# mit-han-lab/distrifuser

Measured on AMD Instinct MI355X. Metric: end-to-end latency (s) per image, SDXL 50-step DDIM, lower is better.
Workload: dtype bf16; 1 GPU; model=sdxl-base (random init), global_batch=1, image=3840x3840, seq_len=230400, scheduler=ddim, steps_per_image=50, parallelism=patch1, mode=corrected_async_gn, cuda_graph=True

## Files before the change

distrifuser_amd/csrc/bindings.hip:

```cpp

#include <torch/extension.h>
#include <ATen/hip/HIPContext.h>
#include <c10/hip/HIPStream.h>

#include <array>

#include "kernels.h"

namespace {

int dtype_of(const at::Tensor& t) {
    switch (t.scalar_type()) {
        case at::kBFloat16: return DFA_BF16;
        case at::kHalf: return DFA_F16;
        case at::kFloat: return DFA_F32;
        default: TORCH_CHECK(false, "unsupported dtype ", t.scalar_type());
    }
}

bool is_b16(const at::Tensor& t) {
    return t.scalar_type() == at::kBFloat16 || t.scalar_type() == at::kHalf;
}

hipStream_t cur_stream() { return at::hip::getCurrentHIPStream().stream(); }

at::Tensor b16_param(const at::Tensor& t, const at::Tensor& ref, const char* op,
                     const char* name) {
    TORCH_CHECK(t.scalar_type() == ref.scalar_type() || !is_b16(t), op, ": ", name,
                " must have x's dtype (", ref.scalar_type(), "), got ", t.scalar_type());
    return t.to(ref.scalar_type()).contiguous();
}

at::Tensor gn_partial_stats(const at::Tensor& x, int64_t group_len, int ngt) {
    auto partial = at::zeros({2, (long)ngt}, x.options().dtype(at::kFloat));
    launch_gn_stats_partial(x.data_ptr(), partial.data_ptr<float>(), group_len, ngt,
                            dtype_of(x), cur_stream());
    return partial;
}

const void* gn_affine(const c10::optional<at::Tensor>& t, const at::Tensor& x, at::Tensor& keep) {
    if (!t.has_value()) return nullptr;
    keep = t->to(x.scalar_type()).contiguous();
    return keep.data_ptr();
}

at::Tensor group_norm_stats(const at::Tensor& x_, int64_t num_groups) {
    TORCH_CHECK(x_.is_cuda() && x_.dim() == 4, "x must be CUDA [N,C,H,W]");
    auto x = x_.contiguous();
    const int64_t n = x.size(0), c = x.size(1), hw = x.size(2) * x.size(3);
    TORCH_CHECK(c % num_groups == 0);
    const int64_t group_len = (c / num_groups) * hw;
    const int ngt = (int)(n * num_groups);
    auto partial = gn_partial_stats(x, group_len, ngt);
    auto out = at::empty({2, n, num_groups, 1, 1, 1}, x.options());
    launch_gn_finalize(partial.data_ptr<float>(), out.data_ptr(), 1.0f / (float)group_len, ngt,
                       dtype_of(x), cur_stream());
    return out;
}

at::Tensor group_norm_apply(const at::Tensor& x_, const at::Tensor& mean_,
                            const at::Tensor& meansq_, const c10::optional<at::Tensor>& w_,
                            const c10::optional<at::Tensor>& b_, double eps, bool silu) {
    TORCH_CHECK(x_.is_cuda() && x_.dim() == 4);
    auto x = x_.contiguous();
    const int64_t n = x.size(0), c = x.size(1), hw = x.size(2) * x.size(3);
    auto mean = mean_.to(at::kFloat).contiguous().view({-1});
    auto meansq = meansq_.to(at::kFloat).contiguous().view({-1});
    TORCH_CHECK(mean.numel() % n == 0);
    const int g = (int)(mean.numel() / n);
    TORCH_CHECK(c % g == 0, "channels ", c, " not divisible by groups ", g);
    at::Tensor w, b;
    const void* wp = gn_affine(w_, x, w);
    const void* bp = gn_affine(b_, x, b);
    auto y = at::empty_like(x);
    launch_gn_apply(x.data_ptr(), y.data_ptr(), mean.data_ptr<float>(), meansq.data_ptr<float>(),
                    wp, bp, (float)eps, hw, (int)c, g, (int)n, silu, dtype_of(x), cur_stream());
    return y;
}

at::Tensor group_norm_silu(const at::Tensor& x_, int64_t num_groups,
                           const c10::optional<at::Tensor>& w_,
                           const c10::optional<at::Tensor>& b_, double eps, bool silu) {
    TORCH_CHECK(x_.is_cuda() && x_.dim() == 4);
    auto x = x_.contiguous();
    const int64_t n = x.size(0), c = x.size(1), hw = x.size(2) * x.size(3);
    TORCH_CHECK(c % num_groups == 0);
    const int64_t group_len = (c / num_groups) * hw;
    const int ngt = (int)(n * num_groups);
    auto partial = gn_partial_stats(x, group_len, ngt);
    auto moments = at::empty({2, (long)ngt}, x.options().dtype(at::kFloat));
    launch_gn_finalize(partial.data_ptr<float>(), moments.data_ptr(), 1.0f / (float)group_len,
                       ngt, DFA_F32, cur_stream());
    at::Tensor w, b;
    const void* wp = gn_affine(w_, x, w);
    const void* bp = gn_affine(b_, x, b);
    auto y = at::empty_like(x);
    launch_gn_apply(x.data_ptr(), y.data_ptr(), moments.data_ptr<float>(),
                    moments.data_ptr<float>() + ngt, wp, bp, (float)eps, hw, (int)c,
                    (int)num_groups, (int)n, silu, dtype_of(x), cur_stream());
    return y;
}

at::Tensor gn_merge_stats(const at::Tensor& buffer, int64_t slot_off, int64_t own,
                          const at::Tensor& fresh_, bool corrected) {
    TORCH_CHECK(buffer.is_cuda() && buffer.dim() == 2 && buffer.stride(1) == 1);
    auto fresh = fresh_.contiguous();
    const int ng = (int)(fresh.numel() / 2);
    TORCH_CHECK(fresh.scalar_type() == buffer.scalar_type());
    auto out = at::empty({2, (long)ng}, buffer.options().dtype(at::kFloat));
    launch_gn_merge_stats(buffer.data_ptr(), buffer.stride(0), slot_off,
                          (int)buffer.size(0), (int)own, fresh.data_ptr(),
                          out.data_ptr<float>(), ng, corrected, dtype_of(buffer),
                          cur_stream());
    return out;
}

at::Tensor geglu(const at::Tensor& h_) {
    TORCH_CHECK(h_.is_cuda());
    auto h = h_.contiguous();
    const int64_t inner = h.size(-1) / 2;
    TORCH_CHECK(h.size(-1) % 2 == 0);
    auto sizes = h.sizes().vec();
    sizes.back() = inner;
    auto out = at::empty(sizes, h.options());
    launch_geglu(h.data_ptr(), out.data_ptr(), h.numel() / (2 * inner), inner, dtype_of(h),
                 cur_stream());
    return out;
}

at::Tensor cfg_affine_step(const at::Tensor& noise, const at::Tensor& x, double g, double ca,
                           double cb) {
    TORCH_CHECK(noise.is_cuda() && noise.size(0) == 2);
    auto n = noise.contiguous();
// ... 334 lines not shown
    p.k = reinterpret_cast<const uint16_t*>(kc.data_ptr());
    p.v = reinterpret_cast<const uint16_t*>(vc.data_ptr());
    p.B = (int)qc.size(0);
    p.L = qc.size(1);
    p.sb = qc.stride(0);
    p.scale = 1.0f / std::sqrt(512.0f);
    auto o = at::empty_like(qc);
    p.o = reinterpret_cast<uint16_t*>(o.data_ptr());
    launch_vae_attention(p, dtype_of(q), cur_stream());
    return o;
}

std::vector<at::Tensor> mfma_probe(const at::Tensor& a, const at::Tensor& b) {
    TORCH_CHECK(a.is_cuda() && a.sizes() == (at::IntArrayRef{64, 8}));
    auto af = a.to(at::kFloat).contiguous(), bf = b.to(at::kFloat).contiguous();
    auto d = at::zeros({64, 4}, af.options());
    launch_mfma_probe(af.data_ptr<float>(), bf.data_ptr<float>(), d.data_ptr<float>(),
                      cur_stream());
    return {d};
}

std::vector<at::Tensor> mfma_probe32(const at::Tensor& a, const at::Tensor& b) {
    TORCH_CHECK(a.is_cuda() && a.sizes() == (at::IntArrayRef{64, 8}));
    auto af = a.to(at::kFloat).contiguous(), bf = b.to(at::kFloat).contiguous();
    auto d = at::zeros({64, 16}, af.options());
    launch_mfma_probe32(af.data_ptr<float>(), bf.data_ptr<float>(), d.data_ptr<float>(),
                        cur_stream());
    return {d};
}
}

PYBIND11_MODULE(TORCH_EXTENSION_NAME, m) {
    m.def("group_norm_stats", &group_norm_stats, "per-group moments [2,N,G,1,1,1]");
    m.def("group_norm_apply", &group_norm_apply, "normalize+affine(+SiLU) from given moments");
    m.def("group_norm_silu", &group_norm_silu, "fused GroupNorm(+SiLU)");
    m.def("geglu", &geglu, "a * gelu(gate) over last-dim halves");
    m.def("gn_merge_stats", &gn_merge_stats,
          "merge stale peer GN moments with fresh local ones (one launch)");
    m.def("cfg_affine_step", &cfg_affine_step, "fused CFG combine + affine scheduler update");
    m.def("flash_attention", &flash_attention, "bf16/fp16 flash attention (chunked stale KV)");
    m.def("flash_attention_ext", &flash_attention_ext,
          "flash attention with split-KV and optional log-sum-exp -> [out] or [out, lse]",
          pybind11::arg("q"), pybind11::arg("k"), pybind11::arg("v"),
          pybind11::arg("kv_splits") = 1, pybind11::arg("return_lse") = false);
    m.def("flash_attention_partial", &flash_attention_partial,
          "split-KV partials into caller buffers (o_part fp32 [S,B,Lq,H,D], lse_part [S,B,H,Lq])");
    m.def("merge_attention", &merge_attention,
          "merge fp32 attention partials by their log-sum-exp -> [out, lse]",
          pybind11::arg("o_parts"), pybind11::arg("lse_parts"), pybind11::arg("out_bf16") = true,
          pybind11::arg("out_dtype") = pybind11::none());
    m.def("cfg_dpm_step", &cfg_dpm_step, "fused CFG + DPM-Solver++(2M) update -> (prev, x0)");
    m.def("layer_norm", &layer_norm, "bf16/fp16 fused LayerNorm");
    m.def("add_layer_norm", &add_layer_norm, "bf16/fp16 fused residual-add + LayerNorm -> (sum, y)");
    m.def("vae_attention", &vae_attention, "bf16/fp16 single-head d=512 VAE mid attention");
    m.def("conv3x3", &conv3x3,
          "bf16/fp16 implicit-GEMM 3x3 conv, stride 1/2, in-place halo rows; pad_lo=0 "
          "(stride 2) pads bottom/right only",
          pybind11::arg("x"), pybind11::arg("wp"), pybind11::arg("bias"), pybind11::arg("cout"), pybind11::arg("stride"),
          pybind11::arg("top"), pybind11::arg("bot"), pybind11::arg("residual"), pybind11::arg("bias2"),
          pybind11::arg("pad_lo") = 1);
    m.def("mfma_probe", &mfma_probe, "dump mfma_f32_16x16x32_bf16 fragment mapping");
    m.def("mfma_probe32", &mfma_probe32, "dump mfma_f32_32x32x16_bf16 fragment mapping");
}
```

distrifuser_amd/csrc/groupnorm.hip:

```cpp

#include "common.h"
#include "kernels.h"
#include <algorithm>

namespace {

template <typename T, bool VEC>
__global__ void gn_stats_partial_kernel(const T* __restrict__ x, float* __restrict__ partial,
                                        int64_t group_len, int chunks, int ngt) {
    constexpr int V = VEC ? VecN<T>::value : 1;
    const int ng = blockIdx.x / chunks;
    const int chunk = blockIdx.x % chunks;
    const int64_t nvec = group_len / V;
    const int64_t per = (nvec + chunks - 1) / chunks;
    const int64_t v0 = chunk * per;
    const int64_t v1 = min(v0 + per, nvec);
    const T* base = x + (int64_t)ng * group_len;

    float s = 0.f, ss = 0.f;
    for (int64_t iv = v0 + threadIdx.x; iv < v1; iv += blockDim.x) {
        if (VEC) {
            uint4 raw = *reinterpret_cast<const uint4*>(base + iv * V);
            const T* e = reinterpret_cast<const T*>(&raw);
#pragma unroll
            for (int j = 0; j < V; ++j) {
                float f = to_f32(e[j]);
                s += f;
                ss += f * f;
            }
        } else {
            float f = to_f32(base[iv]);
            s += f;
            ss += f * f;
// ... 73 lines not shown
        gn_stats_partial_kernel<T, true><<<grid, 256, 0, stream>>>(
            reinterpret_cast<const T*>(x), partial, group_len, chunks, ngt);
    else
        gn_stats_partial_kernel<T, false><<<grid, 256, 0, stream>>>(
            reinterpret_cast<const T*>(x), partial, group_len, chunks, ngt);
}

template <typename T>
void gn_apply_t(const void* x, void* y, const float* mean, const float* meansq, const void* w,
                const void* b, float eps, int64_t hw, int C, int G, int N, bool silu,
                hipStream_t stream) {
    const int64_t total = (int64_t)N * C * hw;
    const bool vec = (hw % VecN<T>::value) == 0;
    const int block = 256;
    if (vec) {
        int grid = grid_for(total / VecN<T>::value, block);
        if (silu)
            gn_apply_kernel<T, true, true><<<grid, block, 0, stream>>>(
                (const T*)x, (T*)y, mean, meansq, (const T*)w, (const T*)b, eps, hw, C, G, total);
        else
            gn_apply_kernel<T, false, true><<<grid, block, 0, stream>>>(
                (const T*)x, (T*)y, mean, meansq, (const T*)w, (const T*)b, eps, hw, C, G, total);
    } else {
        int grid = grid_for(total, block);
        if (silu)
            gn_apply_kernel<T, true, false><<<grid, block, 0, stream>>>(
                (const T*)x, (T*)y, mean, meansq, (const T*)w, (const T*)b, eps, hw, C, G, total);
        else
            gn_apply_kernel<T, false, false><<<grid, block, 0, stream>>>(
                (const T*)x, (T*)y, mean, meansq, (const T*)w, (const T*)b, eps, hw, C, G, total);
    }
}

template <typename T, bool CORRECTED>
__global__ void gn_merge_stats_kernel(T* __restrict__ buffer, int64_t row_stride,
                                      int64_t slot_off, int n_peers, int own,
                                      const T* __restrict__ fresh, float* __restrict__ out,
                                      int ng) {
    const int g = blockIdx.x * blockDim.x + threadIdx.x;
    if (g >= ng) return;
    float m_sum = 0.f, q_sum = 0.f;
    float m_own = 0.f, q_own = 0.f;
    for (int p = 0; p < n_peers; ++p) {
        const T* slot = buffer + p * row_stride + slot_off;
        float m = to_f32(slot[g]);
        float q = to_f32(slot[ng + g]);
        if (p == own) {
            m_own = m;
            q_own = q;
            if (!CORRECTED) {
                m = to_f32(fresh[g]);
                q = to_f32(fresh[ng + g]);
            }
        }
        m_sum += m;
        q_sum += q;
    }
    float mean = m_sum / n_peers;
    float msq = q_sum / n_peers;
    const float f_m = to_f32(fresh[g]);
    const float f_q = to_f32(fresh[ng + g]);
    if (CORRECTED) {
        mean += f_m - m_own;
        msq += f_q - q_own;
        const float var = msq - mean * mean;
        if (var < 0.f) msq = mean * mean + (f_q - f_m * f_m);
// ... 58 lines not shown
void launch_gn_finalize(const float* partial, void* out, float inv_count, int ngt, int dtype,
                        hipStream_t stream) {
    int total = 2 * ngt;
    int block = 256;
    int grid = (total + block - 1) / block;
    switch (dtype) {
        case DFA_BF16:
            gn_finalize_kernel<bf16_t><<<grid, block, 0, stream>>>(partial, (bf16_t*)out, inv_count, ngt);
            break;
        case DFA_F16:
            gn_finalize_kernel<f16_t><<<grid, block, 0, stream>>>(partial, (f16_t*)out, inv_count, ngt);
            break;
        default:
            gn_finalize_kernel<float><<<grid, block, 0, stream>>>(partial, (float*)out, inv_count, ngt);
            break;
    }
}

void launch_gn_apply(const void* x, void* y, const float* mean, const float* meansq,
                     const void* weight, const void* bias, float eps, int64_t hw, int C, int G,
                     int N, bool silu, int dtype, hipStream_t stream) {
    switch (dtype) {
        case DFA_BF16:
            gn_apply_t<bf16_t>(x, y, mean, meansq, weight, bias, eps, hw, C, G, N, silu, stream);
            break;
        case DFA_F16:
            gn_apply_t<f16_t>(x, y, mean, meansq, weight, bias, eps, hw, C, G, N, silu, stream);
            break;
        default:
            gn_apply_t<float>(x, y, mean, meansq, weight, bias, eps, hw, C, G, N, silu, stream);
            break;
    }
}
```

distrifuser_amd/csrc/kernels.h:

```cpp
#pragma once

#include <hip/hip_runtime.h>
#include <cstdint>

enum DfaDtype : int { DFA_BF16 = 0, DFA_F16 = 1, DFA_F32 = 2 };

void launch_gn_stats_partial(const void* x, float* partial, int64_t group_len,
                             int n_groups_total, int dtype, hipStream_t stream);
void launch_gn_finalize(const float* partial, void* out, float inv_count,
                        int n_groups_total, int dtype, hipStream_t stream);
void launch_gn_apply(const void* x, void* y, const float* mean, const float* meansq,
                     const void* weight, const void* bias, float eps, int64_t hw,
                     int C, int G, int N, bool silu, int dtype, hipStream_t stream);

void launch_gn_merge_stats(void* buffer, int64_t row_stride, int64_t slot_off,
                           int n_peers, int own, const void* fresh, float* out,
                           int ng, bool corrected, int dtype, hipStream_t stream);

void launch_geglu(const void* in, void* out, int64_t rows, int64_t inner, int dtype,
                  hipStream_t stream);

void launch_cfg_affine_step(const void* noise_u, const void* noise_c, const void* x, void* out,
                            float g, float ca, float cb, int64_t total, int dtype,
                            hipStream_t stream);

struct Conv3x3Params {
    const uint16_t* x;
    const uint16_t* top;
    const uint16_t* bot;
    const uint16_t* wp;
    const uint16_t* bias;
    const uint16_t* residual;
    const uint16_t* bias2;
    uint16_t* o;
    int B, Cin, Cout, H, W, Ho, Wo;
    int KS, CT;
    int debug;
    int pad_lo;
    int64_t x_sb, x_sc;
    int64_t t_sb, t_sc;
    int64_t b_sb, b_sc;
};
void launch_conv3x3(const Conv3x3Params& p, int stride, int dtype, hipStream_t stream);

void launch_cfg_dpm_step(const void* nu, const void* nc, const void* x, const void* x0_prev,
                         void* out, void* x0_out, float g, float ca, float cb, float cc,
// ... 53 lines not shown
```

distrifuser_amd/models/transformer.py:

```python

from __future__ import annotations

import torch
from torch import nn

from .. import ops

from .layers import LayerFactory


class BasicTransformerBlock(nn.Module):
    def __init__(
        self,
        dim: int,
        heads: int,
        dim_head: int,
        cross_dim: int,
        *,
        factory: LayerFactory,
    ):
        super().__init__()
        self.norm1 = nn.LayerNorm(dim)
        self.attn1 = factory.self_attention(dim, heads, dim_head)
        self.norm2 = nn.LayerNorm(dim)
        self.attn2 = factory.cross_attention(dim, cross_dim, heads, dim_head)
        self.norm3 = nn.LayerNorm(dim)
        self.ff = factory.feed_forward(dim)

    def forward(self, x: torch.Tensor, encoder_hidden_states: torch.Tensor,
                pending=None):
        if pending is None:
            n1 = ops.layer_norm(x, self.norm1.weight, self.norm1.bias, self.norm1.eps)
        else:
            x, n1 = ops.add_layer_norm(x, pending, self.norm1.weight, self.norm1.bias,
                                       self.norm1.eps)
        x, h = ops.add_layer_norm(x, self.attn1(n1), self.norm2.weight, self.norm2.bias,
                                  self.norm2.eps)
        x, n3 = ops.add_layer_norm(x, self.attn2(h, encoder_hidden_states),
                                   self.norm3.weight, self.norm3.bias, self.norm3.eps)
        return x, self.ff(n3)


class Transformer2DModel(nn.Module):

    def __init__(
        self,
        channels: int,
        heads: int,
        dim_head: int,
        layers: int,
        cross_dim: int,
        *,
        factory: LayerFactory,
        groups: int = 32,
        use_linear_projection: bool = True,
    ):
        super().__init__()
        inner = heads * dim_head
        self.use_linear_projection = use_linear_projection
        self.norm = factory.group_norm(groups, channels, eps=1e-6, fuse_silu=False)
        if use_linear_projection:
            self.proj_in = nn.Linear(channels, inner)
            self.proj_out = nn.Linear(inner, channels)
        else:
            self.proj_in = nn.Conv2d(channels, inner, 1)
            self.proj_out = nn.Conv2d(inner, channels, 1)
        self.transformer_blocks = nn.ModuleList(
            [
                BasicTransformerBlock(inner, heads, dim_head, cross_dim, factory=factory)
                for _ in range(layers)
            ]
        )

    def forward(self, x: torch.Tensor, encoder_hidden_states: torch.Tensor) -> torch.Tensor:
        b, c, h, w = x.shape
        residual = x
        x = self.norm(x)
        if self.use_linear_projection:
            x = x.permute(0, 2, 3, 1).reshape(b, h * w, c)
            x = self.proj_in(x)
        else:
            x = self.proj_in(x)
            inner = x.shape[1]
            x = x.permute(0, 2, 3, 1).reshape(b, h * w, inner)
        import os
        if os.environ.get("DFA_NO_PENDING_CHAIN", "0") == "1":
            for block in self.transformer_blocks:
                x, p = block(x, encoder_hidden_states, None)
                x = x + p
        else:
            pending = None
            for block in self.transformer_blocks:
                x, pending = block(x, encoder_hidden_states, pending)
            x = x + pending
        if self.use_linear_projection:
            x = self.proj_out(x)
            x = x.reshape(b, h, w, c).permute(0, 3, 1, 2)
        else:
            inner = x.shape[-1]
            x = x.reshape(b, h, w, inner).permute(0, 3, 1, 2)
            x = self.proj_out(x)
        return x + residual
```

distrifuser_amd/ops/__init__.py:

```python

from .conv import NativeConv2d, conv3x3_halo, pack_conv3x3_weight
from .dispatch import (
    add_layer_norm,
    attention_kv_splits,
    flash_attention,
    flash_attention_chunked,
    geglu,
    group_norm_apply,
    group_norm_silu,
    group_norm_stats,
    hip_ext,
    hip_ext_available,
    layer_norm,
    merge_attention,
    vae_attention,
)
from .norm import PlainGroupNorm

__all__ = [
    "NativeConv2d",
    "PlainGroupNorm",
    "add_layer_norm",
    "attention_kv_splits",
    "layer_norm",
    "conv3x3_halo",
    "flash_attention",
    "flash_attention_chunked",
    "geglu",
    "group_norm_apply",
    "group_norm_silu",
    "group_norm_stats",
    "hip_ext",
    "hip_ext_available",
    "merge_attention",
    "pack_conv3x3_weight",
    "vae_attention",
]
```

distrifuser_amd/ops/dispatch.py:

```python

from __future__ import annotations

import os

import torch

from . import eager

_EXT = None
_EXT_ERR: Exception | None = None


def _force_eager() -> bool:
    return os.environ.get("DFA_FORCE_EAGER", "0") == "1"


def hip_ext():
    global _EXT, _EXT_ERR
    if _EXT is not None or _EXT_ERR is not None:
        if _EXT is None:
            raise RuntimeError(f"distrifuser_amd HIP extension failed to load: {_EXT_ERR}")
        return _EXT
    try:
        import importlib
# ... 138 lines not shown
    *,
    multi_processor_count: int | None = None,
) -> int:
    if dim_head > 64 or min(b, heads, lq, lkv) <= 0:
        return 1
    cus = multi_processor_count
    if cus is None:
        cus = _DEFAULT_CUS
        if torch.cuda.is_available() and (device is None or torch.device(device).type == "cuda"):
            cus = torch.cuda.get_device_properties(device).multi_processor_count
    blocks = -(-lq // _Q_BLOCK) * b * heads
    tiles = -(-lkv // _KV_TILE)
    if blocks >= cus * _BLOCKS_PER_CU:
        return 1
    part_bytes = 2 * 4 * b * heads * lq * dim_head

    def cost(s: int) -> float:
        t = _TILE_US * -(-tiles // s) * -(-blocks * s // cus)
        if s > 1:
            t += _MERGE_LAUNCH_US + s * part_bytes / _MERGE_BYTES_PER_US
        return t

    s_max = max(1, min(_MAX_KV_SPLITS, tiles // _MIN_TILES_PER_SPLIT))
    best = min((s for s in (1, 2, 4, 8) if s <= s_max), key=cost)
    return best if cost(best) < (1.0 - _MIN_GAIN) * cost(1) else 1


def group_norm_stats(x: torch.Tensor, num_groups: int) -> torch.Tensor:
    if _use_hip(x):
        return hip_ext().group_norm_stats(x, num_groups)
    return eager.group_norm_stats(x, num_groups)


def group_norm_apply(x, mean, meansq, weight, bias, eps, silu=False):
    if _use_hip(x):
        n = x.shape[0]
        g = mean.reshape(n, -1).shape[1]
        return hip_ext().group_norm_apply(
            x,
            mean.reshape(n, g).contiguous(),
            meansq.reshape(n, g).contiguous(),
            weight,
            bias,
            eps,
            silu,
        )
    return eager.group_norm_apply(x, mean, meansq, weight, bias, eps, silu)


def group_norm_silu(x, num_groups, weight, bias, eps, silu=True):
    if _use_hip(x):
        return hip_ext().group_norm_silu(x, num_groups, weight, bias, eps, silu)
    return eager.group_norm_silu(x, num_groups, weight, bias, eps, silu)


def layer_norm(x, weight, bias, eps):
    if _use_hip(x) and x.dtype in _KERNEL_DTYPES and x.shape[-1] % 8 == 0 and x.shape[-1] <= 2048:
        return hip_ext().layer_norm(x, weight, bias, eps)
    return eager.layer_norm(x, weight, bias, eps)


def add_layer_norm(x, res, weight, bias, eps):
    if _use_hip(x) and x.dtype in _KERNEL_DTYPES and x.shape[-1] % 8 == 0 and x.shape[-1] <= 2048:
        s, y = hip_ext().add_layer_norm(x, res, weight, bias, eps)
        return s, y
    return eager.add_layer_norm(x, res, weight, bias, eps)


def vae_attention(q: torch.Tensor, k: torch.Tensor, v: torch.Tensor) -> torch.Tensor:
    if _use_hip(q) and q.dtype in _KERNEL_DTYPES and q.shape[-1] == 512:
        return hip_ext().vae_attention(q, k, v)
    return eager.vae_attention(q, k, v)


def geglu(hidden: torch.Tensor) -> torch.Tensor:
    if _use_hip(hidden):
        return hip_ext().geglu(hidden)
    return eager.geglu(hidden)
```

distrifuser_amd/ops/eager.py:

```python

from __future__ import annotations

import torch
import torch.nn.functional as F


def flash_attention(q: torch.Tensor, k: torch.Tensor, v: torch.Tensor) -> torch.Tensor:
    return F.scaled_dot_product_attention(q, k, v, dropout_p=0.0, is_causal=False)


def flash_attention_lse(
    q: torch.Tensor, k: torch.Tensor, v: torch.Tensor
) -> tuple[torch.Tensor, torch.Tensor]:
    scores = torch.einsum("bhqd,bhkd->bhqk", q.float(), k.float()) * q.shape[-1] ** -0.5
    lse = torch.logsumexp(scores, dim=-1)
    probs = torch.exp(scores - lse.unsqueeze(-1))
    out = torch.einsum("bhqk,bhkd->bhqd", probs, v.float())
    return out.to(q.dtype), lse


def merge_attention(
    o_parts: torch.Tensor, lse_parts: torch.Tensor, out_dtype: torch.dtype | None = None
) -> tuple[torch.Tensor, torch.Tensor]:
    lse_f = lse_parts.float()
    m = lse_f.max(dim=0).values
    empty = torch.isneginf(m)
    w = torch.exp(lse_f - torch.where(empty, torch.zeros_like(m), m))
    wsum = w.sum(dim=0)
    wq = w.permute(0, 1, 3, 2).unsqueeze(-1)
    acc = torch.where(wq > 0, wq * o_parts.float(), torch.zeros((), device=w.device)).sum(dim=0)
    denom = torch.where(empty, torch.ones_like(wsum), wsum).permute(0, 2, 1).unsqueeze(-1)
    out = acc / denom
    lse = torch.where(empty, m, m + torch.log(wsum))
    return out.to(o_parts.dtype if out_dtype is None else out_dtype), lse


def group_norm_stats(x: torch.Tensor, num_groups: int) -> torch.Tensor:
    n, c, h, w = x.shape
    xg = x.reshape(n, num_groups, -1).float()
    mean = xg.mean(dim=-1)
    meansq = (xg * xg).mean(dim=-1)
    return torch.stack([mean, meansq], dim=0).reshape(2, n, num_groups, 1, 1, 1).to(x.dtype)


def group_norm_apply(
    x: torch.Tensor,
    mean: torch.Tensor,
    meansq: torch.Tensor,
    weight: torch.Tensor | None,
    bias: torch.Tensor | None,
    eps: float,
    silu: bool = False,
) -> torch.Tensor:
    n, c, h, w = x.shape
    g = mean.reshape(n, -1).shape[1]
    mean = mean.reshape(n, g, 1).float()
    meansq = meansq.reshape(n, g, 1).float()
    var = (meansq - mean * mean).clamp_min_(0.0)
    inv_std = torch.rsqrt(var + eps)
    out = (x.reshape(n, g, -1).float() - mean) * inv_std
    out = out.reshape(n, c, h, w)
    if weight is not None:
        out = out * weight.float().view(1, -1, 1, 1)
    if bias is not None:
        out = out + bias.float().view(1, -1, 1, 1)
    if silu:
        out = F.silu(out)
    return out.to(x.dtype)


def group_norm_silu(
    x: torch.Tensor,
    num_groups: int,
    weight: torch.Tensor | None,
    bias: torch.Tensor | None,
    eps: float,
    silu: bool = True,
) -> torch.Tensor:
    out = F.group_norm(x.float(), num_groups, None if weight is None else weight.float(),
                       None if bias is None else bias.float(), eps)
    if silu:
        out = F.silu(out)
    return out.to(x.dtype)


def geglu(hidden: torch.Tensor) -> torch.Tensor:
    a, b = hidden.chunk(2, dim=-1)
    return a * F.gelu(b)


def layer_norm(x, weight, bias, eps):
    import torch.nn.functional as _F

    return _F.layer_norm(x, (x.shape[-1],), weight, bias, eps)


def add_layer_norm(x, res, weight, bias, eps):
    import torch.nn.functional as _F

    s = x + res
    return s, _F.layer_norm(s, (s.shape[-1],), weight, bias, eps)


def vae_attention(q: torch.Tensor, k: torch.Tensor, v: torch.Tensor) -> torch.Tensor:
    scale = q.shape[-1] ** -0.5
    scores = torch.einsum("bqc,bkc->bqk", q.float() * scale, k.float())
    probs = scores.softmax(dim=-1)
    return torch.einsum("bqk,bkc->bqc", probs, v.float()).to(q.dtype)


def conv3x3_halo(
    x: torch.Tensor,
    weight: torch.Tensor,
    bias: torch.Tensor | None,
    stride: int = 1,
    top: torch.Tensor | None = None,
# ... 27 lines not shown
```

distrifuser_amd/ops/norm.py:

```python

from __future__ import annotations

import torch
from torch import nn

from . import dispatch


class PlainGroupNorm(nn.GroupNorm):

    def __init__(self, num_groups, num_channels, eps=1e-5, affine=True, fuse_silu=False):
        super().__init__(num_groups, num_channels, eps=eps, affine=affine)
        self.fuse_silu = fuse_silu

    def forward(self, x: torch.Tensor) -> torch.Tensor:
        return dispatch.group_norm_silu(
            x, self.num_groups, self.weight, self.bias, self.eps, silu=self.fuse_silu
        )
```

distrifuser_amd/parallel/patch_ops.py:

```python

from __future__ import annotations

import os

import torch
import torch.distributed as dist
import torch.nn.functional as F
from torch import nn

from .. import ops
from .state import ParallelState


def _is_patch_parallel(state: ParallelState) -> bool:
    return state.config.parallelism == "patch" and state.config.n_device_per_batch > 1


class PatchConv2d(nn.Module):

    def __init__(
        self,
        in_channels: int,
        out_channels: int,
        kernel_size: int = 3,
# ... 116 lines not shown

class PatchGroupNorm(nn.Module):

    def __init__(
        self,
        num_groups: int,
        num_channels: int,
        eps: float = 1e-5,
        affine: bool = True,
        *,
        state: ParallelState,
        fuse_silu: bool = False,
    ):
        super().__init__()
        self.num_groups = num_groups
        self.num_channels = num_channels
        self.eps = eps
        self.affine = affine
        self.fuse_silu = fuse_silu
        if affine:
            self.weight = nn.Parameter(torch.ones(num_channels))
            self.bias = nn.Parameter(torch.zeros(num_channels))
        else:
            self.register_parameter("weight", None)
            self.register_parameter("bias", None)
        self.state = state
        self._idx: int | None = None
        self._buffer_list: list[torch.Tensor] | None = None

    def reset(self) -> None:
        self._idx = None
        self._buffer_list = None

    def _local(self, x: torch.Tensor) -> torch.Tensor:
        return ops.group_norm_silu(
            x, self.num_groups, self.weight, self.bias, self.eps, silu=self.fuse_silu
        )

    def forward(self, x: torch.Tensor) -> torch.Tensor:
        state = self.state
        cfg = state.config
        if not _is_patch_parallel(state):
            return self._local(x)
        mode = cfg.mode

        if mode in ("separate_gn", "no_sync"):
            return self._local(x)

        if mode in ("sync_gn", "full_sync"):
            stats = ops.group_norm_stats(x, self.num_groups)
            dist.all_reduce(stats, op=dist.ReduceOp.SUM, group=cfg.batch_group)
            stats = stats / cfg.n_device_per_batch
            return ops.group_norm_apply(
                x, stats[0], stats[1], self.weight, self.bias, self.eps, silu=self.fuse_silu
            )

        assert mode in ("stale_gn", "corrected_async_gn")
        comm = state.comm_manager
        n, c, h, w = x.shape

        if self._buffer_list is None:
            if comm is None or comm.buffer is None:
                if comm is not None and state.recording and self._idx is None:
                    self._idx = comm.register_tensor(
                        (2, n, self.num_groups, 1, 1, 1), x.dtype, layer_type="gn"
                    )
                return self._local(x)
            if self._idx is None:
                return self._local(x)
            self._buffer_list = comm.get_buffer_list(self._idx)

        comm.wait(self._idx)
        fresh = ops.group_norm_stats(x, self.num_groups)

        if not state.in_warmup and x.is_cuda and not os.environ.get("DFA_FORCE_EAGER") == "1":
            moments = ops.hip_ext().gn_merge_stats(
                comm.buffer, comm.starts[self._idx], cfg.split_idx(), fresh,
                mode == "corrected_async_gn",
            )
            comm.enqueue(self._idx)
            return ops.group_norm_apply(
                x, moments[0], moments[1], self.weight, self.bias, self.eps,
                silu=self.fuse_silu,
            )

        if state.in_warmup:
            dist.all_gather(self._buffer_list, fresh, group=cfg.batch_group)
            full = torch.stack(self._buffer_list).float().mean(dim=0)
        elif mode == "corrected_async_gn":
            stale_own = self._buffer_list[cfg.split_idx()]
            full = torch.stack(self._buffer_list).float().mean(dim=0) + (
                fresh.float() - stale_own.float()
            )
            comm.enqueue(self._idx, fresh)
        else:
            stack = torch.stack(
                [
                    fresh if p == cfg.split_idx() else buf
                    for p, buf in enumerate(self._buffer_list)
                ]
            )
            full = stack.float().mean(dim=0)
            comm.enqueue(self._idx, fresh)

        mean, meansq = full[0], full[1]
        if mode == "corrected_async_gn" and not state.in_warmup:
            var = meansq - mean * mean
            f_mean, f_meansq = fresh[0].float(), fresh[1].float()
            local_var = f_meansq - f_mean * f_mean
            neg = var < 0
            meansq = torch.where(neg, mean * mean + local_var, meansq)
        return ops.group_norm_apply(
            x, mean, meansq, self.weight, self.bias, self.eps, silu=self.fuse_silu
        )


class PatchSelfAttention(nn.Module):

    def __init__(
        self,
        query_dim: int,
        heads: int,
        dim_head: int,
        out_bias: bool = True,
        *,
        state: ParallelState,
    ):
        super().__init__()
        inner = heads * dim_head
        self.heads = heads
        self.dim_head = dim_head
        self.to_q = nn.Linear(query_dim, inner, bias=False)
        self.to_kv = nn.Linear(query_dim, 2 * inner, bias=False)
        self.to_out = nn.Linear(inner, query_dim, bias=out_bias)
        self.state = state
        self._idx: int | None = None
        self._buffer_view: torch.Tensor | None = None
        self._buffer_list: list[torch.Tensor] | None = None
        self._wqkv: torch.Tensor | None = None
        self._wqkv_key = None

    def reset(self) -> None:
        self._idx = None
        self._buffer_view = None
        self._buffer_list = None

# ... 108 lines not shown
```

Baseline: 28.22 s/image.

## Fuse GroupNorm with NCHW-to-tokens transpose and proj_out residual add

Adds a GroupNorm apply variant that writes its output directly in [N, HW, C] token layout, so the transformer block's proj_in no longer needs a separate permute and contiguous copy. It also adds a kernel that transposes the proj_out result back to NCHW while adding the residual in the same pass. Both use LDS-tiled transposes with swizzled shared memory and 16-byte vector accesses. The aim is to remove extra full-tensor passes over very large activations at 3840x3840, at the cost of more kernel code and a different rounding path for the fused norm.

```diff
diff --git a/distrifuser_amd/csrc/bindings.hip b/distrifuser_amd/csrc/bindings.hip
--- a/distrifuser_amd/csrc/bindings.hip
+++ b/distrifuser_amd/csrc/bindings.hip
@@ -5,6 +5,7 @@
 
 #include <array>
 
+#include "boundary_plan.h"
 #include "kernels.h"
 
 namespace {
@@ -42,6 +43,24 @@
     if (!t.has_value()) return nullptr;
     keep = t->to(x.scalar_type()).contiguous();
     return keep.data_ptr();
+}
+
+at::Tensor gn_apply_out(const at::Tensor& x, const float* mean, const float* meansq,
+                        const void* wp, const void* bp, double eps, int g, bool silu,
+                        bool tokens) {
+    const int64_t n = x.size(0), c = x.size(1), hw = x.size(2) * x.size(3);
+    if (!tokens) {
+        auto y = at::empty_like(x);
+        launch_gn_apply(x.data_ptr(), y.data_ptr(), mean, meansq, wp, bp, (float)eps, hw, (int)c,
+                        g, (int)n, silu, dtype_of(x), cur_stream());
+        return y;
+    }
+    auto y = at::empty({n, hw, c}, x.options());
+    const BoundaryPlan pl = boundary_plan(n, c, hw, (int)x.element_size(), true);
+    TORCH_CHECK(pl.ok || pl.empty, "group_norm tokens: shape too large for one launch");
+    launch_gn_apply_tokens(x.data_ptr(), y.data_ptr(), mean, meansq, wp, bp, (float)eps, hw,
+                           (int)c, g, (int)n, silu, dtype_of(x), cur_stream());
+    return y;
 }
 
 at::Tensor group_norm_stats(const at::Tensor& x_, int64_t num_groups) {
@@ -60,10 +79,11 @@
 
 at::Tensor group_norm_apply(const at::Tensor& x_, const at::Tensor& mean_,
                             const at::Tensor& meansq_, const c10::optional<at::Tensor>& w_,
-                            const c10::optional<at::Tensor>& b_, double eps, bool silu) {
+                            const c10::optional<at::Tensor>& b_, double eps, bool silu,
+                            bool tokens) {
     TORCH_CHECK(x_.is_cuda() && x_.dim() == 4);
     auto x = x_.contiguous();
-    const int64_t n = x.size(0), c = x.size(1), hw = x.size(2) * x.size(3);
+    const int64_t n = x.size(0), c = x.size(1);
     auto mean = mean_.to(at::kFloat).contiguous().view({-1});
     auto meansq = meansq_.to(at::kFloat).contiguous().view({-1});
     TORCH_CHECK(mean.numel() % n == 0);
@@ -72,15 +92,14 @@
     at::Tensor w, b;
     const void* wp = gn_affine(w_, x, w);
     const void* bp = gn_affine(b_, x, b);
-    auto y = at::empty_like(x);
-    launch_gn_apply(x.data_ptr(), y.data_ptr(), mean.data_ptr<float>(), meansq.data_ptr<float>(),
-                    wp, bp, (float)eps, hw, (int)c, g, (int)n, silu, dtype_of(x), cur_stream());
-    return y;
+    return gn_apply_out(x, mean.data_ptr<float>(), meansq.data_ptr<float>(), wp, bp, eps, g, silu,
+                        tokens);
 }
 
 at::Tensor group_norm_silu(const at::Tensor& x_, int64_t num_groups,
                            const c10::optional<at::Tensor>& w_,
-                           const c10::optional<at::Tensor>& b_, double eps, bool silu) {
+                           const c10::optional<at::Tensor>& b_, double eps, bool silu,
+                           bool tokens) {
     TORCH_CHECK(x_.is_cuda() && x_.dim() == 4);
     auto x = x_.contiguous();
     const int64_t n = x.size(0), c = x.size(1), hw = x.size(2) * x.size(3);
@@ -94,11 +113,32 @@
     at::Tensor w, b;
     const void* wp = gn_affine(w_, x, w);
     const void* bp = gn_affine(b_, x, b);
-    auto y = at::empty_like(x);
-    launch_gn_apply(x.data_ptr(), y.data_ptr(), moments.data_ptr<float>(),
-                    moments.data_ptr<float>() + ngt, wp, bp, (float)eps, hw, (int)c,
-                    (int)num_groups, (int)n, silu, dtype_of(x), cur_stream());
-    return y;
+    return gn_apply_out(x, moments.data_ptr<float>(), moments.data_ptr<float>() + ngt, wp, bp, eps,
+                        (int)num_groups, silu, tokens);
+}
+
+at::Tensor tokens_add_nchw(const at::Tensor& y_, const at::Tensor& residual) {
+    TORCH_CHECK(y_.is_cuda() && y_.dim() == 3 && residual.is_cuda() && residual.dim() == 4,
+                "tokens_add_nchw: y [N,HW,C] and residual [N,C,H,W] on the GPU");
+    TORCH_CHECK(y_.scalar_type() == residual.scalar_type(),
+                "tokens_add_nchw: residual must have y's dtype (", y_.scalar_type(), "), got ",
+                residual.scalar_type());
+    const int64_t n = residual.size(0), c = residual.size(1);
+    const int64_t hw = residual.size(2) * residual.size(3);
+    TORCH_CHECK(y_.size(0) == n && y_.size(1) == hw && y_.size(2) == c,
+                "tokens_add_nchw: y must be [N, H*W, C] of residual [N, C, H, W]");
+    const int64_t sizes[4] = {n, c, residual.size(2), residual.size(3)};
+    const int64_t strides[4] = {residual.stride(0), residual.stride(1), residual.stride(2),
+                                residual.stride(3)};
+    TORCH_CHECK(boundary_plane_contiguous(sizes, strides),
+                "tokens_add_nchw: residual's (H, W) plane must be contiguous");
+    auto y = y_.contiguous();
+    auto out = at::empty({n, c, residual.size(2), residual.size(3)}, y.options());
+    const BoundaryPlan pl = boundary_plan(n, c, hw, (int)y.element_size(), true);
+    TORCH_CHECK(pl.ok || pl.empty, "tokens_add_nchw: shape too large for one launch");
+    launch_tokens_add_nchw(y.data_ptr(), residual.data_ptr(), out.data_ptr(), hw, (int)c, (int)n,
+                           strides[0], strides[1], dtype_of(y), cur_stream());
+    return out;
 }
 
 at::Tensor gn_merge_stats(const at::Tensor& buffer, int64_t slot_off, int64_t own,
@@ -499,8 +539,17 @@
 
 PYBIND11_MODULE(TORCH_EXTENSION_NAME, m) {
     m.def("group_norm_stats", &group_norm_stats, "per-group moments [2,N,G,1,1,1]");
-    m.def("group_norm_apply", &group_norm_apply, "normalize+affine(+SiLU) from given moments");
-    m.def("group_norm_silu", &group_norm_silu, "fused GroupNorm(+SiLU)");
+    m.def("group_norm_apply", &group_norm_apply,
+          "normalize+affine(+SiLU) from given moments; tokens: write [N, HW, C]",
+          pybind11::arg("x"), pybind11::arg("mean"), pybind11::arg("meansq"),
+          pybind11::arg("weight"), pybind11::arg("bias"), pybind11::arg("eps"),
+          pybind11::arg("silu"), pybind11::arg("tokens") = false);
+    m.def("group_norm_silu", &group_norm_silu, "fused GroupNorm(+SiLU); tokens: write [N, HW, C]",
+          pybind11::arg("x"), pybind11::arg("num_groups"), pybind11::arg("weight"),
+          pybind11::arg("bias"), pybind11::arg("eps"), pybind11::arg("silu"),
+          pybind11::arg("tokens") = false);
+    m.def("tokens_add_nchw", &tokens_add_nchw,
+          "y [N, HW, C] + residual [N, C, H, W] -> [N, C, H, W] (transposing residual add)");
     m.def("geglu", &geglu, "a * gelu(gate) over last-dim halves");
     m.def("gn_merge_stats", &gn_merge_stats,
           "merge stale peer GN moments with fresh local ones (one launch)");
diff --git a/distrifuser_amd/csrc/boundary_plan.h b/distrifuser_amd/csrc/boundary_plan.h
--- /dev/null
+++ b/distrifuser_amd/csrc/boundary_plan.h
@@ -0,0 +1,37 @@
+#pragma once
+
+#include <cstdint>
+
+constexpr int BOUNDARY_VEC_TILE = 64;
+constexpr int BOUNDARY_SCALAR_TILE = 32;
+constexpr int BOUNDARY_THREADS = 256;
+constexpr int64_t BOUNDARY_MAX_GRID_YZ = 65535;
+
+struct BoundaryPlan {
+    bool ok;
+    bool empty;
+    bool vec;
+    int tile;
+    int64_t grid_x, grid_y, grid_z;
+};
+
+inline BoundaryPlan boundary_plan(int64_t n, int64_t c, int64_t hw, int elem_size,
+                                  bool aligned16) {
+    BoundaryPlan p{};
+    if (n < 0 || c < 0 || hw < 0) return p;
+    p.empty = n == 0 || c == 0 || hw == 0;
+    p.vec = elem_size == 2 && aligned16 && hw % 8 == 0 && c % 8 == 0;
+    p.tile = p.vec ? BOUNDARY_VEC_TILE : BOUNDARY_SCALAR_TILE;
+    p.grid_x = (hw + p.tile - 1) / p.tile;
+    p.grid_y = (c + p.tile - 1) / p.tile;
+    p.grid_z = n;
+    p.ok = !p.empty && p.grid_x <= INT32_MAX && p.grid_y <= BOUNDARY_MAX_GRID_YZ &&
+           p.grid_z <= BOUNDARY_MAX_GRID_YZ;
+    return p;
+}
+
+inline bool boundary_plane_contiguous(const int64_t sizes[4], const int64_t strides[4]) {
+    const bool w_ok = sizes[3] <= 1 || strides[3] == 1;
+    const bool h_ok = sizes[2] <= 1 || strides[2] == sizes[3];
+    return w_ok && h_ok;
+}
diff --git a/distrifuser_amd/csrc/groupnorm.hip b/distrifuser_amd/csrc/groupnorm.hip
--- a/distrifuser_amd/csrc/groupnorm.hip
+++ b/distrifuser_amd/csrc/groupnorm.hip
@@ -1,4 +1,5 @@
 
+#include "boundary_plan.h"
 #include "common.h"
 #include "kernels.h"
 #include <algorithm>
@@ -138,6 +139,265 @@
     }
 }
 
+constexpr int BT = BOUNDARY_VEC_TILE;
+
+__device__ __forceinline__ int bt_dword(int prow, int cp) {
+    return prow * (BT / 2) + (((cp >> 2) ^ ((prow >> 3) & 7)) << 2 | (cp & 3));
+}
+__device__ __forceinline__ int bt_chunk(int prow, int q) {
+    return prow * (BT / 2) + ((q ^ ((prow >> 3) & 7)) << 2);
+}
+
+template <typename T>
+__device__ __forceinline__ uint32_t bits16(T v) {
+    return (uint32_t)__builtin_bit_cast(uint16_t, v);
+}
+
+template <bool FUSED>
+__device__ __forceinline__ void gn_scale_shift(float m, float msq, float eps, float wv, float bv,
+                                               float& sc, float& sh) {
+#pragma clang fp contract(off)
+    float var = __builtin_fmaf(-m, m, msq);
+    var = var < 0.f ? 0.f : var;
+    const float inv = rsqrtf(var + eps);
+    sc = wv * inv;
+    if (FUSED) {
+        sh = __builtin_fmaf(-m, sc, bv);
+    } else {
+        const float ms = m * sc;
+        sh = bv - ms;
+    }
+}
+template <bool FUSED>
+__device__ __forceinline__ float gn_norm(float x, float sc, float sh) {
+#pragma clang fp contract(off)
+    if (FUSED) return __builtin_fmaf(x, sc, sh);
+    const float xs = x * sc;
+    return xs + sh;
+}
+
+template <typename T, bool SILU>
+__global__ __launch_bounds__(BOUNDARY_THREADS) void gn_apply_tokens_vec_kernel(
+    const T* __restrict__ x, T* __restrict__ y, const float* __restrict__ mean,
+    const float* __restrict__ meansq, const T* __restrict__ w, const T* __restrict__ b, float eps,
+    int64_t hw, int C, int G) {
+    static_assert(sizeof(T) == 2, "16-bit types only");
+    __shared__ __attribute__((aligned(16))) uint32_t tile[BT * BT / 2];
+    const int t = threadIdx.x;
+    const int64_t n = blockIdx.z;
+    const int c0 = blockIdx.y * BT;
+    const int64_t p0 = (int64_t)blockIdx.x * BT;
+    const int gs = C / G;
+    {
+        const int pv = t & 7, cp = t >> 3;
+        const int c = c0 + 2 * cp;
+        const int64_t p = p0 + pv * 8;
+        uint32_t packed[8] = {0, 0, 0, 0, 0, 0, 0, 0};
+        if (c < C && p < hw) {
+#pragma unroll
+            for (int h = 0; h < 2; ++h) {
+                const int ch = c + h;
+                const int g = ch / gs;
+                float sc, sh;
+                gn_scale_shift<true>(mean[n * G + g], meansq[n * G + g], eps,
+                                     w ? to_f32(w[ch]) : 1.f, b ? to_f32(b[ch]) : 0.f, sc, sh);
+                const uint4 raw = *reinterpret_cast<const uint4*>(x + (n * C + ch) * hw + p);
+                const T* e = reinterpret_cast<const T*>(&raw);
+#pragma unroll
+                for (int j = 0; j < 8; ++j) {
+                    float f = gn_norm<true>(to_f32(e[j]), sc, sh);
+                    if (SILU) f = siluf(f);
+                    packed[j] |= bits16(from_f32<T>(f)) << (16 * h);
+                }
+            }
+        }
+#pragma unroll
+        for (int j = 0; j < 8; ++j) tile[bt_dword(pv * 8 + j, cp)] = packed[j];
+    }
+    __syncthreads();
+    {
+        const int q = t & 7;
+        const int ch = c0 + q * 8;
+#pragma unroll
+        for (int pass = 0; pass < 2; ++pass) {
+            const int pr = (t >> 3) + 32 * pass;
+            const int64_t pix = p0 + pr;
+            const uint4 v = *reinterpret_cast<const uint4*>(&tile[bt_chunk(pr, q)]);
+            if (pix < hw && ch < C) *reinterpret_cast<uint4*>(y + (n * hw + pix) * C + ch) = v;
+        }
+    }
+}
+
+template <typename T, bool SILU, bool FUSED>
+__global__ __launch_bounds__(BOUNDARY_THREADS) void gn_apply_tokens_scalar_kernel(
+    const T* __restrict__ x, T* __restrict__ y, const float* __restrict__ mean,
+    const float* __restrict__ meansq, const T* __restrict__ w, const T* __restrict__ b, float eps,
+    int64_t hw, int C, int G) {
+    constexpr int S = BOUNDARY_SCALAR_TILE;
+    __shared__ float tile[S][S + 1];
+    const int tx = threadIdx.x & 31, ty = threadIdx.x >> 5;
+    const int64_t n = blockIdx.z;
+    const int c0 = blockIdx.y * S;
+    const int64_t p0 = (int64_t)blockIdx.x * S;
+    const int gs = C / G;
+#pragma unroll
+    for (int i = 0; i < S / 8; ++i) {
+        const int cl = ty + 8 * i;
+        const int c = c0 + cl;
+        const int64_t p = p0 + tx;
+        if (c < C && p < hw) {
+            const int g = c / gs;
+            float sc, sh;
+            gn_scale_shift<FUSED>(mean[n * G + g], meansq[n * G + g], eps,
+                                  w ? to_f32(w[c]) : 1.f, b ? to_f32(b[c]) : 0.f, sc, sh);
+            float f = gn_norm<FUSED>(to_f32(x[(n * C + c) * hw + p]), sc, sh);
+            if (SILU) f = siluf(f);
+            tile[cl][tx] = f;
+        }
+    }
+    __syncthreads();
+#pragma unroll
+    for (int i = 0; i < S / 8; ++i) {
+        const int pl = ty + 8 * i;
+        const int64_t p = p0 + pl;
+        const int c = c0 + tx;
+        if (c < C && p < hw) y[(n * hw + p) * C + c] = from_f32<T>(tile[tx][pl]);
+    }
+}
+
+template <typename T>
+__global__ __launch_bounds__(BOUNDARY_THREADS) void tokens_add_nchw_vec_kernel(
+    const T* __restrict__ y, const T* __restrict__ res, T* __restrict__ out, int64_t hw, int C,
+    int64_t rs_n, int64_t rs_c) {
+    static_assert(sizeof(T) == 2, "16-bit types only");
+    __shared__ __attribute__((aligned(16))) uint32_t tile[BT * BT / 2];
+    const int t = threadIdx.x;
+    const int64_t n = blockIdx.z;
+    const int c0 = blockIdx.y * BT;
+    const int64_t p0 = (int64_t)blockIdx.x * BT;
+    const int pv = t & 7, cp = t >> 3;
+    const int c = c0 + 2 * cp;
+    const int64_t p = p0 + pv * 8;
+    const bool live = c < C && p < hw;
+    uint4 r[2] = {uint4{0, 0, 0, 0}, uint4{0, 0, 0, 0}};
+    if (live) {
+        r[0] = *reinterpret_cast<const uint4*>(res + n * rs_n + (int64_t)c * rs_c + p);
+        r[1] = *reinterpret_cast<const uint4*>(res + n * rs_n + (int64_t)(c + 1) * rs_c + p);
+    }
+    {
+        const int q = t & 7;
+        const int ch = c0 + q * 8;
+#pragma unroll
+        for (int pass = 0; pass < 2; ++pass) {
+            const int pr = (t >> 3) + 32 * pass;
+            const int64_t pix = p0 + pr;
+            uint4 v{0, 0, 0, 0};
+            if (pix < hw && ch < C) v = *reinterpret_cast<const uint4*>(y + (n * hw + pix) * C + ch);
+            *reinterpret_cast<uint4*>(&tile[bt_chunk(pr, q)]) = v;
+        }
+    }
+    __syncthreads();
+    if (live) {
+        uint32_t d[8];
+#pragma unroll
+        for (int j = 0; j < 8; ++j) d[j] = tile[bt_dword(pv * 8 + j, cp)];
+#pragma unroll
+        for (int h = 0; h < 2; ++h) {
+            const T* re = reinterpret_cast<const T*>(&r[h]);
+            uint4 outv;
+            T* o = reinterpret_cast<T*>(&outv);
+#pragma unroll
+            for (int j = 0; j < 8; ++j) {
+                const T yv = __builtin_bit_cast(T, (uint16_t)(d[j] >> (16 * h)));
+                o[j] = from_f32<T>(to_f32(yv) + to_f32(re[j]));
+            }
+            *reinterpret_cast<uint4*>(out + (n * C + c + h) * hw + p) = outv;
+        }
+    }
+}
+
+template <typename T>
+__global__ __launch_bounds__(BOUNDARY_THREADS) void tokens_add_nchw_scalar_kernel(
+    const T* __restrict__ y, const T* __restrict__ res, T* __restrict__ out, int64_t hw, int C,
+    int64_t rs_n, int64_t rs_c) {
+    constexpr int S = BOUNDARY_SCALAR_TILE;
+    __shared__ float tile[S][S + 1];
+    const int tx = threadIdx.x & 31, ty = threadIdx.x >> 5;
+    const int64_t n = blockIdx.z;
+    const int c0 = blockIdx.y * S;
+    const int64_t p0 = (int64_t)blockIdx.x * S;
+#pragma unroll
+    for (int i = 0; i < S / 8; ++i) {
+        const int pl = ty + 8 * i;
+        const int64_t p = p0 + pl;
+        const int c = c0 + tx;
+        if (c < C && p < hw) tile[pl][tx] = to_f32(y[(n * hw + p) * C + c]);
+    }
+    __syncthreads();
+#pragma unroll
+    for (int i = 0; i < S / 8; ++i) {
+        const int cl = ty + 8 * i;
+        const int c = c0 + cl;
+        const int64_t p = p0 + tx;
+        if (c < C && p < hw)
+            out[(n * C + c) * hw + p] =
+                from_f32<T>(tile[tx][cl] + to_f32(res[n * rs_n + (int64_t)c * rs_c + p]));
+    }
+}
+
+inline bool aligned16(const void* p) { return (reinterpret_cast<uintptr_t>(p) & 15) == 0; }
+
+template <typename T>
+void gn_apply_tokens_t(const void* x, void* y, const float* mean, const float* meansq,
+                       const void* w, const void* b, float eps, int64_t hw, int C, int G, int N,
+                       bool silu, hipStream_t stream) {
+    const BoundaryPlan pl =
+        boundary_plan(N, C, hw, (int)sizeof(T), aligned16(x) && aligned16(y));
+    if (!pl.ok) return;
+    const dim3 grid((unsigned)pl.grid_x, (unsigned)pl.grid_y, (unsigned)pl.grid_z);
+#define DFA_GN_TOKENS_LAUNCH(...)                                                            \
+    __VA_ARGS__<<<grid, BOUNDARY_THREADS, 0, stream>>>((const T*)x, (T*)y, mean, meansq,     \
+                                                       (const T*)w, (const T*)b, eps, hw, C, G)
+    if constexpr (sizeof(T) == 2) {
+        if (pl.vec) {
+            if (silu)
+                DFA_GN_TOKENS_LAUNCH(gn_apply_tokens_vec_kernel<T, true>);
+            else
+                DFA_GN_TOKENS_LAUNCH(gn_apply_tokens_vec_kernel<T, false>);
+            return;
+        }
+    }
+    const bool fused = (hw % VecN<T>::value) == 0;
+    if (silu && fused)
+        DFA_GN_TOKENS_LAUNCH(gn_apply_tokens_scalar_kernel<T, true, true>);
+    else if (silu)
+        DFA_GN_TOKENS_LAUNCH(gn_apply_tokens_scalar_kernel<T, true, false>);
+    else if (fused)
+        DFA_GN_TOKENS_LAUNCH(gn_apply_tokens_scalar_kernel<T, false, true>);
+    else
+        DFA_GN_TOKENS_LAUNCH(gn_apply_tokens_scalar_kernel<T, false, false>);
+#undef DFA_GN_TOKENS_LAUNCH
+}
+
+template <typename T>
+void tokens_add_nchw_t(const void* y, const void* res, void* out, int64_t hw, int C, int N,
+                       int64_t rs_n, int64_t rs_c, hipStream_t stream) {
+    const bool al = aligned16(y) && aligned16(res) && aligned16(out) && rs_n % 8 == 0 &&
+                    rs_c % 8 == 0;
+    const BoundaryPlan pl = boundary_plan(N, C, hw, (int)sizeof(T), al);
+    if (!pl.ok) return;
+    const dim3 grid((unsigned)pl.grid_x, (unsigned)pl.grid_y, (unsigned)pl.grid_z);
+    if constexpr (sizeof(T) == 2) {
+        if (pl.vec) {
+            tokens_add_nchw_vec_kernel<T><<<grid, BOUNDARY_THREADS, 0, stream>>>(
+                (const T*)y, (const T*)res, (T*)out, hw, C, rs_n, rs_c);
+            return;
+        }
+    }
+    tokens_add_nchw_scalar_kernel<T><<<grid, BOUNDARY_THREADS, 0, stream>>>(
+        (const T*)y, (const T*)res, (T*)out, hw, C, rs_n, rs_c);
+}
+
 template <typename T, bool CORRECTED>
 __global__ void gn_merge_stats_kernel(T* __restrict__ buffer, int64_t row_stride,
                                       int64_t slot_off, int n_peers, int own,
@@ -262,3 +522,41 @@
             break;
     }
 }
+
+void launch_gn_apply_tokens(const void* x, void* y, const float* mean, const float* meansq,
+                            const void* weight, const void* bias, float eps, int64_t hw, int C,
+                            int G, int N, bool silu, int dtype, hipStream_t stream) {
+    switch (dtype) {
+        case DFA_BF16:
+            gn_apply_tokens_t<bf16_t>(x, y, mean, meansq, weight, bias, eps, hw, C, G, N, silu,
+                                      stream);
+            break;
+        case DFA_F16:
+            gn_apply_tokens_t<f16_t>(x, y, mean, meansq, weight, bias, eps, hw, C, G, N, silu,
+                                     stream);
+            break;
+        default:
+            gn_apply_tokens_t<float>(x, y, mean, meansq, weight, bias, eps, hw, C, G, N, silu,
+                                     stream);
+            break;
+    }
+}
+
+void launch_tokens_add_nchw(const void* y, const void* residual, void* out, int64_t hw, int C,
+                            int N, int64_t res_stride_n, int64_t res_stride_c, int dtype,
+                            hipStream_t stream) {
+    switch (dtype) {
+        case DFA_BF16:
+            tokens_add_nchw_t<bf16_t>(y, residual, out, hw, C, N, res_stride_n, res_stride_c,
+                                      stream);
+            break;
+        case DFA_F16:
+            tokens_add_nchw_t<f16_t>(y, residual, out, hw, C, N, res_stride_n, res_stride_c,
+                                     stream);
+            break;
+        default:
+            tokens_add_nchw_t<float>(y, residual, out, hw, C, N, res_stride_n, res_stride_c,
+                                     stream);
+            break;
+    }
+}
diff --git a/distrifuser_amd/csrc/kernels.h b/distrifuser_amd/csrc/kernels.h
--- a/distrifuser_amd/csrc/kernels.h
+++ b/distrifuser_amd/csrc/kernels.h
@@ -12,6 +12,14 @@
 void launch_gn_apply(const void* x, void* y, const float* mean, const float* meansq,
                      const void* weight, const void* bias, float eps, int64_t hw,
                      int C, int G, int N, bool silu, int dtype, hipStream_t stream);
+
+void launch_gn_apply_tokens(const void* x, void* y, const float* mean, const float* meansq,
+                            const void* weight, const void* bias, float eps, int64_t hw,
+                            int C, int G, int N, bool silu, int dtype, hipStream_t stream);
+
+void launch_tokens_add_nchw(const void* y, const void* residual, void* out, int64_t hw, int C,
+                            int N, int64_t res_stride_n, int64_t res_stride_c, int dtype,
+                            hipStream_t stream);
 
 void launch_gn_merge_stats(void* buffer, int64_t row_stride, int64_t slot_off,
                            int n_peers, int own, const void* fresh, float* out,
diff --git a/distrifuser_amd/models/transformer.py b/distrifuser_amd/models/transformer.py
--- a/distrifuser_amd/models/transformer.py
+++ b/distrifuser_amd/models/transformer.py
@@ -1,5 +1,7 @@
 
 from __future__ import annotations
+
+import os
 
 import torch
 from torch import nn
@@ -58,6 +60,9 @@
         super().__init__()
         inner = heads * dim_head
         self.use_linear_projection = use_linear_projection
+        self.boundary_fuse = (
+            use_linear_projection and os.environ.get("DFA_NO_BOUNDARY_FUSE", "0") != "1"
+        )
         self.norm = factory.group_norm(groups, channels, eps=1e-6, fuse_silu=False)
         if use_linear_projection:
             self.proj_in = nn.Linear(channels, inner)
@@ -75,15 +80,18 @@
     def forward(self, x: torch.Tensor, encoder_hidden_states: torch.Tensor) -> torch.Tensor:
         b, c, h, w = x.shape
         residual = x
-        x = self.norm(x)
-        if self.use_linear_projection:
+        if self.boundary_fuse:
+            x = self.norm(x, tokens=True)
+            x = torch.matmul(x, self.proj_in.weight.t()).add_(self.proj_in.bias)
+        elif self.use_linear_projection:
+            x = self.norm(x)
             x = x.permute(0, 2, 3, 1).reshape(b, h * w, c)
             x = self.proj_in(x)
         else:
+            x = self.norm(x)
             x = self.proj_in(x)
             inner = x.shape[1]
             x = x.permute(0, 2, 3, 1).reshape(b, h * w, inner)
-        import os
         if os.environ.get("DFA_NO_PENDING_CHAIN", "0") == "1":
             for block in self.transformer_blocks:
                 x, p = block(x, encoder_hidden_states, None)
@@ -93,6 +101,8 @@
             for block in self.transformer_blocks:
                 x, pending = block(x, encoder_hidden_states, pending)
             x = x + pending
+        if self.boundary_fuse:
+            return ops.tokens_add_nchw(self.proj_out(x), residual)
         if self.use_linear_projection:
             x = self.proj_out(x)
             x = x.reshape(b, h, w, c).permute(0, 3, 1, 2)
diff --git a/distrifuser_amd/ops/__init__.py b/distrifuser_amd/ops/__init__.py
--- a/distrifuser_amd/ops/__init__.py
+++ b/distrifuser_amd/ops/__init__.py
@@ -13,6 +13,7 @@
     hip_ext_available,
     layer_norm,
     merge_attention,
+    tokens_add_nchw,
     vae_attention,
 )
 from .norm import PlainGroupNorm
@@ -34,5 +35,6 @@
     "hip_ext_available",
     "merge_attention",
     "pack_conv3x3_weight",
+    "tokens_add_nchw",
     "vae_attention",
 ]
diff --git a/distrifuser_amd/ops/dispatch.py b/distrifuser_amd/ops/dispatch.py
--- a/distrifuser_amd/ops/dispatch.py
+++ b/distrifuser_amd/ops/dispatch.py
@@ -194,7 +194,7 @@
     return eager.group_norm_stats(x, num_groups)
 
 
-def group_norm_apply(x, mean, meansq, weight, bias, eps, silu=False):
+def group_norm_apply(x, mean, meansq, weight, bias, eps, silu=False, tokens=False):
     if _use_hip(x):
         n = x.shape[0]
         g = mean.reshape(n, -1).shape[1]
@@ -206,14 +206,32 @@
             bias,
             eps,
             silu,
+            tokens,
         )
-    return eager.group_norm_apply(x, mean, meansq, weight, bias, eps, silu)
-
-
-def group_norm_silu(x, num_groups, weight, bias, eps, silu=True):
+    return eager.group_norm_apply(x, mean, meansq, weight, bias, eps, silu, tokens)
+
+
+def group_norm_silu(x, num_groups, weight, bias, eps, silu=True, tokens=False):
     if _use_hip(x):
-        return hip_ext().group_norm_silu(x, num_groups, weight, bias, eps, silu)
-    return eager.group_norm_silu(x, num_groups, weight, bias, eps, silu)
+        return hip_ext().group_norm_silu(x, num_groups, weight, bias, eps, silu, tokens)
+    return eager.group_norm_silu(x, num_groups, weight, bias, eps, silu, tokens)
+
+
+_BOUNDARY_DTYPES = (torch.bfloat16, torch.float16, torch.float32)
+
+
+def tokens_add_nchw(y: torch.Tensor, residual: torch.Tensor) -> torch.Tensor:
+    if (
+        _use_hip(y)
+        and y.dtype in _BOUNDARY_DTYPES
+        and residual.dtype == y.dtype
+        and residual.is_cuda
+        and residual.dim() == 4
+        and (residual.shape[3] <= 1 or residual.stride(3) == 1)
+        and (residual.shape[2] <= 1 or residual.stride(2) == residual.shape[3])
+    ):
+        return hip_ext().tokens_add_nchw(y, residual)
+    return eager.tokens_add_nchw(y, residual)
 
 
 def layer_norm(x, weight, bias, eps):
diff --git a/distrifuser_amd/ops/eager.py b/distrifuser_amd/ops/eager.py
--- a/distrifuser_amd/ops/eager.py
+++ b/distrifuser_amd/ops/eager.py
@@ -43,6 +43,16 @@
     return torch.stack([mean, meansq], dim=0).reshape(2, n, num_groups, 1, 1, 1).to(x.dtype)
 
 
+def nchw_to_tokens(x: torch.Tensor) -> torch.Tensor:
+    n, c, h, w = x.shape
+    return x.permute(0, 2, 3, 1).reshape(n, h * w, c).contiguous()
+
+
+def tokens_add_nchw(y: torch.Tensor, residual: torch.Tensor) -> torch.Tensor:
+    n, c, h, w = residual.shape
+    return (y.reshape(n, h, w, c).permute(0, 3, 1, 2) + residual).contiguous()
+
+
 def group_norm_apply(
     x: torch.Tensor,
     mean: torch.Tensor,
@@ -51,6 +61,7 @@
     bias: torch.Tensor | None,
     eps: float,
     silu: bool = False,
+    tokens: bool = False,
 ) -> torch.Tensor:
     n, c, h, w = x.shape
     g = mean.reshape(n, -1).shape[1]
@@ -66,7 +77,8 @@
         out = out + bias.float().view(1, -1, 1, 1)
     if silu:
         out = F.silu(out)
-    return out.to(x.dtype)
+    out = out.to(x.dtype)
+    return nchw_to_tokens(out) if tokens else out
 
 
 def group_norm_silu(
@@ -76,12 +88,14 @@
     bias: torch.Tensor | None,
     eps: float,
     silu: bool = True,
+    tokens: bool = False,
 ) -> torch.Tensor:
     out = F.group_norm(x.float(), num_groups, None if weight is None else weight.float(),
                        None if bias is None else bias.float(), eps)
     if silu:
         out = F.silu(out)
-    return out.to(x.dtype)
+    out = out.to(x.dtype)
+    return nchw_to_tokens(out) if tokens else out
 
 
 def geglu(hidden: torch.Tensor) -> torch.Tensor:
diff --git a/distrifuser_amd/ops/norm.py b/distrifuser_amd/ops/norm.py
--- a/distrifuser_amd/ops/norm.py
+++ b/distrifuser_amd/ops/norm.py
@@ -13,7 +13,8 @@
         super().__init__(num_groups, num_channels, eps=eps, affine=affine)
         self.fuse_silu = fuse_silu
 
-    def forward(self, x: torch.Tensor) -> torch.Tensor:
+    def forward(self, x: torch.Tensor, tokens: bool = False) -> torch.Tensor:
         return dispatch.group_norm_silu(
-            x, self.num_groups, self.weight, self.bias, self.eps, silu=self.fuse_silu
+            x, self.num_groups, self.weight, self.bias, self.eps, silu=self.fuse_silu,
+            tokens=tokens,
         )
diff --git a/distrifuser_amd/parallel/patch_ops.py b/distrifuser_amd/parallel/patch_ops.py
--- a/distrifuser_amd/parallel/patch_ops.py
+++ b/distrifuser_amd/parallel/patch_ops.py
@@ -172,27 +172,29 @@
         self._idx = None
         self._buffer_list = None
 
-    def _local(self, x: torch.Tensor) -> torch.Tensor:
+    def _local(self, x: torch.Tensor, tokens: bool = False) -> torch.Tensor:
         return ops.group_norm_silu(
-            x, self.num_groups, self.weight, self.bias, self.eps, silu=self.fuse_silu
-        )
-
-    def forward(self, x: torch.Tensor) -> torch.Tensor:
+            x, self.num_groups, self.weight, self.bias, self.eps, silu=self.fuse_silu,
+            tokens=tokens,
+        )
+
+    def forward(self, x: torch.Tensor, tokens: bool = False) -> torch.Tensor:
         state = self.state
         cfg = state.config
         if not _is_patch_parallel(state):
-            return self._local(x)
+            return self._local(x, tokens)
         mode = cfg.mode
 
         if mode in ("separate_gn", "no_sync"):
-            return self._local(x)
+            return self._local(x, tokens)
 
         if mode in ("sync_gn", "full_sync"):
             stats = ops.group_norm_stats(x, self.num_groups)
             dist.all_reduce(stats, op=dist.ReduceOp.SUM, group=cfg.batch_group)
             stats = stats / cfg.n_device_per_batch
             return ops.group_norm_apply(
-                x, stats[0], stats[1], self.weight, self.bias, self.eps, silu=self.fuse_silu
+                x, stats[0], stats[1], self.weight, self.bias, self.eps, silu=self.fuse_silu,
+                tokens=tokens,
             )
 
         assert mode in ("stale_gn", "corrected_async_gn")
@@ -205,9 +207,9 @@
                     self._idx = comm.register_tensor(
                         (2, n, self.num_groups, 1, 1, 1), x.dtype, layer_type="gn"
                     )
-                return self._local(x)
+                return self._local(x, tokens)
             if self._idx is None:
-                return self._local(x)
+                return self._local(x, tokens)
             self._buffer_list = comm.get_buffer_list(self._idx)
 
         comm.wait(self._idx)
@@ -221,7 +223,7 @@
             comm.enqueue(self._idx)
             return ops.group_norm_apply(
                 x, moments[0], moments[1], self.weight, self.bias, self.eps,
-                silu=self.fuse_silu,
+                silu=self.fuse_silu, tokens=tokens,
             )
 
         if state.in_warmup:
@@ -251,7 +253,8 @@
             neg = var < 0
             meansq = torch.where(neg, mean * mean + local_var, meansq)
         return ops.group_norm_apply(
-            x, mean, meansq, self.weight, self.bias, self.eps, silu=self.fuse_silu
+            x, mean, meansq, self.weight, self.bias, self.eps, silu=self.fuse_silu,
+            tokens=tokens,
         )
 
 
```

After: 27.28 s/image, median of 6. 3.3% less time.
